# PhilippBongartz/RepeatResolver

Hardware: AMD Instinct MI355X
Metric: sum-of-pairs DP cells/sec (higher is better)
Workload: dtype u32

## Files before the change

repeatresolver_amd/csrc/pwr_device.hip:

```cpp
#include <hip/hip_runtime.h>

#include <algorithm>
#include <chrono>
#include <cstdint>
#include <cstdio>
#include <cstdlib>
#include <cstring>
#include <new>
#include <thread>
#include <type_traits>
#include <vector>

#include "pwr.h"

#define PWR_INF 0x40000000u
#define PWR_BIG 0x7fffffff

struct Hdr {
    int W;
    int nslots;
    int nfree;
    int cur;
    int status;
    int stop;
// ... 85 lines not shown
    int fin, active;
    int grow0;
    unsigned long long cells;
};
struct GatherPart;
struct CommitJob {
    int nchg, nev, ndel, first;
    int u0, u1;
    int scanned, pad;
};
struct BatchPlan;
struct CommitEv;
struct JobBufs {
    GatherPart *gpart;
    unsigned gather_tag;
    JobMeta *meta;
    int *way;
    int4 *rec2;
    uint8_t *mark;
    uint8_t *mark2;
    uint32_t *dirs;
    int *newcol;
    int *aux;
    uint4 *desc;
    int wpNW, wpMS;
    unsigned *lastM;
    unsigned long long *gmb;
    SegDesc *seg;
    unsigned *chk;
    int seg_align;
    int src_start;
    int smax, seg_rows, warm_cols;
    int seg_budget, seg_minrows;
    int seg_balance;
    int plan_ahead;
    int hard_rows, hard_up, hard_down;
    int plan_len;
    int plan_gate_rel;
    int spec_inorder;
    int fail_stops;
    int plan_slack, plan_evrate_x100;
    const int *rowids;
    int gstride;
    unsigned tagbase;
    unsigned long long *gtr;
    int trk;
    unsigned trace_tag;
    long long *g64;
    int force64;
    int evcap;
    int gate_v2;
    int *chkdone;
    int check_in_trace, trace_ny;
    int trace_blk;
    int v2_follows, f64_follows;
    int stall_test;
    unsigned long long *diag;
    int njobs_launched;
    int Lmax, colcap, NC;
    size_t dirstride;
    int split_rank, split_world;
    CommitJob *cjob;
    int *chg;
    int *evkey, *evdl;
    int *insidx;
    int *pair_cf, *pair_left;
    BatchPlan *plan;
    CommitEv *sev;
    int *freed;
    unsigned *ticket;
};
#define NOT_MINE(JB, JOB) ((JB).split_world > 1 && (JOB) % (JB).split_world != (JB).split_rank)

#define DPP_ROW_SHR(n) (0x110 + (n))
#define DPP_ROW_BCAST15 0x142
#define DPP_ROW_BCAST31 0x143
#define DPP_WAVE_SHR1 0x138

__device__ __forceinline__ int wave_incl_min(int v)
{
    int t;
    t = __builtin_amdgcn_update_dpp(PWR_BIG, v, DPP_ROW_SHR(1), 0xF, 0xF, false); v = min(v, t);
    t = __builtin_amdgcn_update_dpp(PWR_BIG, v, DPP_ROW_SHR(2), 0xF, 0xF, false); v = min(v, t);
    t = __builtin_amdgcn_update_dpp(PWR_BIG, v, DPP_ROW_SHR(4), 0xF, 0xF, false); v = min(v, t);
    t = __builtin_amdgcn_update_dpp(PWR_BIG, v, DPP_ROW_SHR(8), 0xF, 0xF, false); v = min(v, t);
    t = __builtin_amdgcn_update_dpp(PWR_BIG, v, DPP_ROW_BCAST15, 0xA, 0xF, false); v = min(v, t);
    t = __builtin_amdgcn_update_dpp(PWR_BIG, v, DPP_ROW_BCAST31, 0xC, 0xF, false); v = min(v, t);
    return v;
}
__device__ __forceinline__ int row_incl_min(int v)
{
    int t;
    t = __builtin_amdgcn_update_dpp(PWR_BIG, v, DPP_ROW_SHR(1), 0xF, 0xF, false); v = min(v, t);
    t = __builtin_amdgcn_update_dpp(PWR_BIG, v, DPP_ROW_SHR(2), 0xF, 0xF, false); v = min(v, t);
    t = __builtin_amdgcn_update_dpp(PWR_BIG, v, DPP_ROW_SHR(4), 0xF, 0xF, false); v = min(v, t);
    t = __builtin_amdgcn_update_dpp(PWR_BIG, v, DPP_ROW_SHR(8), 0xF, 0xF, false); v = min(v, t);
    return v;
}
__device__ __forceinline__ unsigned wave_incl_add(unsigned v)
{
    unsigned t;
    t = __builtin_amdgcn_update_dpp(0u, v, DPP_ROW_SHR(1), 0xF, 0xF, false); v += t;
    t = __builtin_amdgcn_update_dpp(0u, v, DPP_ROW_SHR(2), 0xF, 0xF, false); v += t;
    t = __builtin_amdgcn_update_dpp(0u, v, DPP_ROW_SHR(4), 0xF, 0xF, false); v += t;
    t = __builtin_amdgcn_update_dpp(0u, v, DPP_ROW_SHR(8), 0xF, 0xF, false); v += t;
    t = __builtin_amdgcn_update_dpp(0u, v, DPP_ROW_BCAST15, 0xA, 0xF, false); v += t;
// ... 2075 lines not shown
            const int nv = cbit ? (yy << 1) : ((yy << 1) | 1);
            if (phase == 1 && x >= xrec_lo) cnt -= __builtin_amdgcn_readlane(ncreg, x & 63) & 1;
            cnt += nv & 1;
            ncreg = (lane == (x & 63)) ? nv : ncreg;
            yireg = (lane == (x & 63)) ? y : yireg;
            y = cbit ? yy - 1 : yy;
            --x;
            if (x >= 0 && y < 0) { err = 3; break; }
        }
        if (blk * 64 + lane < L && (x < x_top)) { newcol[blk * 64 + lane] = ncreg; yin[blk * 64 + lane] = yireg; }
        if (phase == 0) {
            if (top) {
                if (err) break;
            } else {
                xrec_lo = err ? x + 1 : x_lo;
                if (err == 0) yout_guess = y;
                err = 0;
            }
            if (top) { yout_guess = y; }
        } else {
            if (err) break;
            if (merged && xrec_lo > x_lo) { err = 6; break; }
            if (merged) y = yout_guess;
            yout_guess = y;
        }
    }
    if (lane == 0)
        __hip_atomic_store(&hand[wv], TR_WORD(ttag, err ? 2 : 1, cnt, yout_guess), __ATOMIC_RELAXED, __HIP_MEMORY_SCOPE_AGENT);
    if (err) {
        if (lane == 0) { m->ok = 0; atomicCAS(&st.hdr->status, 0, PWR_ERR_INTERNAL); }
        return;
    }
#ifdef PWR_DIAG
    if (job == 0 && lane == 0 && (wv == 0 || top)) {
        const unsigned long long n_ = __builtin_amdgcn_s_memrealtime();
        unsigned long long *d_ = st.hdr->dbg + (top ? 20 : 16);
        d_[0] += (top ? n_ : tr_t1) - tr_t0; d_[1] += tr_t2 - tr_t1; d_[2] += n_ - (top ? n_ : tr_t2); d_[3] += 1;
    }
#endif
    if (wv == 0 && lane == 0) {
        int tot = cnt;
        for (int c = 1; c < nch; ++c)
            tot += (int)((__hip_atomic_load(&hand[c], __ATOMIC_RELAXED, __HIP_MEMORY_SCOPE_AGENT) >> 24) & 0xffffull);
        m->nnew = tot;
        m->changed = 1;
    }
}

#define TB_W 4
#ifndef TB_C
#define TB_C 32
#endif
#define TB_BROKE 0x1fffffu
#define TB_WORD(TAG, FLAG, CNT, ARR, EXF) (((unsigned long long)((TAG) & 0x3fffu) << 50) | ((unsigned long long)(FLAG) << 48) | ((unsigned long long)((CNT) & 0x7f) << 41) | \
                                           ((unsigned long long)(((ARR) + 1) & 0xfffff) << 21) | (unsigned long long)((EXF) & 0x1fffffu))
#define TB_MAXCOL ((1 << 20) - 4)
__global__ __launch_bounds__(TB_W * 64) void k_trace_blk(DState st, JobBufs jb)
{
    const int job = blockIdx.x, tid = threadIdx.x, lane = tid & 63;
    if (jb.check_in_trace && (int)blockIdx.y >= jb.trace_ny) { seg_check_body(st, jb, job, (int)blockIdx.y - jb.trace_ny + 1, tid); return; }
    JobMeta *m = &jb.meta[job];
    const int L = UNI(m->L);
    if (!m->active || L <= 0 || !m->ok || m->abort || (!jb.check_in_trace && m->segfail) || (m->wide && !jb.f64_follows) || NOT_MINE(jb, job)) return;
    const int nch = (L + TB_C - 1) / TB_C;
    const int c = nch - 1 - UNI((int)blockIdx.y * TB_W + (tid >> 6));
    if (c < 0) return;
    unsigned long long *const hand = jb.gtr + (size_t)job * jb.trk;
    const unsigned ttag = jb.trace_tag & 0x3fffu;
    const int W = UNI(m->W), B = st.B, H = st.H, RS = jb.NC, lo = UNI(m->lo);
    const int *way = jb.way + (size_t)job * jb.Lmax;
    const uint32_t *dirs = jb.dirs + (size_t)job * jb.dirstride;
    const unsigned *lastM = jb.lastM + (size_t)job * jb.NC;
    int *newcol = jb.newcol + (size_t)job * jb.Lmax;
    int *yin = jb.aux + (size_t)job * jb.Lmax;
    const int x_lo = c * TB_C, x_top = min(L, x_lo + TB_C) - 1;
    const bool top = c == nch - 1;
    const int wcur = way[min(x_lo + lane, L - 1)];
    int ncreg = 0, yireg = 0;
    int xrec_lo = x_top + 1;
    int cnt = 0, err = 0, yexit = 0;
    bool broke = false;

    auto pass = [&](int y0, const bool check_merge, bool &merged) __attribute__((always_inline)) {
        int x = x_top, y = y0;
        int gcur = -1, yb = 0;
        uint32_t win[4] = {0, 0, 0, 0};
        int gpre = -1, ybpre = 0;
        uint32_t pre[4] = {0, 0, 0, 0};
        merged = false;
        int e = 0;
        while (x >= x_lo && !e) {
            x = UNI(x); y = UNI(y); gcur = UNI(gcur); yb = UNI(yb); gpre = UNI(gpre); ybpre = UNI(ybpre); cnt = UNI(cnt);
            while ((x >> 4) == gcur && x >= x_lo) {
                if (check_merge && x >= xrec_lo && __builtin_amdgcn_readlane(yireg, x & (TB_C - 1)) == y) { merged = true; break; }
                const int af = max(0, __builtin_amdgcn_readlane(wcur, x & (TB_C - 1)) - H);
                const int ycf = min(y, af + min(B, W - af) - 1);
                if (y < af || ycf < yb || ycf > yb + 255) break;
                const int q0 = (ycf - yb) >> 6, shf = 15 - (x & 15);
                const uint32_t wq = q0 == 0 ? win[0] : q0 == 1 ? win[1] : q0 == 2 ? win[2] : win[3];
                const int cy = yb + 64 * q0 + lane;
                const unsigned long long mk = __ballot(cy <= ycf && cy >= af && !((wq >> shf) & 1u));
                if (!mk) break;
                const int t = 63 - __builtin_clzll(mk);
                const int yy = yb + 64 * q0 + t;
                const int cb = (int)((__ballot((wq >> (16 + shf)) & 1u) >> t) & 1ull);
                const int nv = (yy << 1) | (cb ^ 1);
                if (x >= xrec_lo) cnt -= __builtin_amdgcn_readlane(ncreg, x & (TB_C - 1)) & 1;
                cnt += nv & 1;
                ncreg = (lane == (x & (TB_C - 1))) ? nv : ncreg;
                yireg = (lane == (x & (TB_C - 1))) ? y : yireg;
                y = yy - cb;
                --x;
                if (x >= 0 && y < 0) { e = 3; break; }
            }
            if (merged || e || x < x_lo) break;
            if (check_merge && x >= xrec_lo && __builtin_amdgcn_readlane(yireg, x & (TB_C - 1)) == y) { merged = true; break; }
            const int a = max(0, __builtin_amdgcn_readlane(wcur, x & (TB_C - 1)) - H);
            const int Bx = min(B, W - a);
            if (y < a) { e = 1; break; }
            int yc = min(y, a + Bx - 1);
            const int g = x >> 4, sh = 15 - (x & 15);
            int found = -1, cbit = 0;
            for (;;) {
                if (g != gcur || yc < yb || yc > yb + 255) {
                    if (gpre == g && yc >= ybpre + 96 && yc <= ybpre + 255) {
#pragma unroll
                        for (int q = 0; q < 4; ++q) win[q] = pre[q];
                        yb = ybpre;
                    } else {
                        const int want = max(lo, yc - 191);
#pragma unroll
                        for (int q = 0; q < 4; ++q) win[q] = dirs[(size_t)g * RS + (want + 64 * q + lane - lo) % RS];
                        yb = want;
                    }
                    gcur = g;
                    if (g > (x_lo >> 4)) {
                        gpre = g - 1; ybpre = max(lo, yb - 56);
#pragma unroll
                        for (int q = 0; q < 4; ++q) pre[q] = dirs[(size_t)(g - 1) * RS + (ybpre + 64 * q + lane - lo) % RS];
                    }
                }
                {
                    const int q0 = (yc - yb) >> 6;
                    const uint32_t wq = q0 == 0 ? win[0] : q0 == 1 ? win[1] : q0 == 2 ? win[2] : win[3];
                    const int cy = yb + 64 * q0 + lane;
                    const unsigned long long mk = __ballot(cy <= yc && cy >= a && !((wq >> sh) & 1u));
                    if (mk) {
                        const int t = 63 - __builtin_clzll(mk);
                        found = yb + 64 * q0 + t;
                        const unsigned long long ck = __ballot((wq >> (16 + sh)) & 1u);
                        cbit = (int)((ck >> t) & 1ull);
                    } else {
#pragma unroll
                        for (int q = 2; q >= 0; --q) {
                            if (found < 0 && q < q0) {
                                const int cy2 = yb + 64 * q + lane;
                                const unsigned long long mk2 = __ballot(cy2 >= a && !((win[q] >> sh) & 1u));
                                if (mk2) {
                                    const int t = 63 - __builtin_clzll(mk2);
                                    found = yb + 64 * q + t;
                                    const unsigned long long ck = __ballot((win[q] >> (16 + sh)) & 1u);
                                    cbit = (int)((ck >> t) & 1ull);
                                }
                            }
                        }
                    }
                }
                if (found >= 0) break;
                if (yb <= a) { e = 2; break; }
                yc = yb - 1;
            }
            if (e) break;
            const int yy = found;
            const int nv = cbit ? (yy << 1) : ((yy << 1) | 1);
            if (x >= xrec_lo) cnt -= __builtin_amdgcn_readlane(ncreg, x & (TB_C - 1)) & 1;
            cnt += nv & 1;
            ncreg = (lane == (x & (TB_C - 1))) ? nv : ncreg;
            yireg = (lane == (x & (TB_C - 1))) ? y : yireg;
            y = cbit ? yy - 1 : yy;
            --x;
            if (x >= 0 && y < 0) { e = 3; break; }
        }
        if (!merged) xrec_lo = e ? min(xrec_lo, x + 1) : x_lo;
        if (!e && !merged) yexit = y;
        return e;
    };
#define TB_POST(FLAG, ARR) if (lane == 0) __hip_atomic_store(&hand[c], TB_WORD(ttag, FLAG, cnt, ARR, broke ? TB_BROKE : (unsigned)(yexit + 1)), __ATOMIC_RELAXED, __HIP_MEMORY_SCOPE_AGENT);

    bool merged = false;
#ifdef PWR_DIAG
    const unsigned long long tb_t0 = __builtin_amdgcn_s_memrealtime();
    unsigned long long tb_t1 = tb_t0;
    int tb_looks = 0, tb_retr = 0;
#endif
    if (top) {
        const int wx = UNI(way[L - 1]);
        const int a = max(0, wx - H), Bx = min(B, W - a);
        int ylow = max(-1, wx - H) + 1;
        if (ylow > W - 1) ylow = W - 1;
        unsigned long long key = ~0ull;
        {
            constexpr int EN = (PWR_MAX_BANDWIDTH + 63) / 64;
            const int y0_ = max(ylow, a) + lane;
            unsigned ev[EN];
#pragma unroll
            for (int i = 0; i < EN; ++i) { const int yy = y0_ + 64 * i; ev[i] = yy < a + Bx ? lastM[(yy - lo) % RS] : 0xffffffffu; }
#pragma unroll
            for (int i = 0; i < EN; ++i) {
                const int yy = y0_ + 64 * i;
                const unsigned long long k2 = yy < a + Bx ? (((unsigned long long)ev[i] << 32) | (unsigned)(~(unsigned)yy)) : ~0ull;
                key = k2 < key ? k2 : key;
            }
        }
        for (int o = 32; o > 0; o >>= 1) {
            const unsigned long long other = __shfl_xor(key, o);
            key = other < key ? other : key;
        }
        const unsigned vmin = (unsigned)(key >> 32);
        int entry = (key == ~0ull) ? -1 : (int)(~(unsigned)key);
        if (a + B <= W - 1) {
            const unsigned lastval = lastM[(a + B - 1 - lo) % RS];
            if (entry < 0 || lastval <= vmin) entry = W - 1;
        }
        entry = UNI(entry);
        if (lane == 0) m->entry = entry;
        err = entry < 0 ? 4 : pass(entry, false, merged);
    } else {
        int arr = UNI(way[x_top + 1]) - 1;
        broke = pass(arr, false, merged) != 0;
        TB_POST(1, arr)
#ifdef PWR_DIAG
        tb_t1 = __builtin_amdgcn_s_memrealtime();
#endif
        for (int look = 0; look < (1 << 16) && !err; ++look) {
#ifdef PWR_DIAG
            tb_looks += 1;
#endif
            int t = c + 1;
            int verdict = 0;
            int bad = -1;
// ... 14 lines not shown
                unsigned ex_up = (unsigned)__shfl_down((int)ex_j, 1);
                if (lane == 63) {
                    const int j2 = min(t + 64, nch - 1);
                    int s2 = 0;
                    for (int spin = 0; spin < TR_SPIN_LIMIT; ++spin) {
                        wn = __hip_atomic_load(&hand[j2], __ATOMIC_RELAXED, __HIP_MEMORY_SCOPE_AGENT);
                        s2 = ((unsigned)(wn >> 50) == ttag) ? (int)((wn >> 48) & 3ull) : 0;
                        if (s2) break;
                        __builtin_amdgcn_s_sleep(1);
                    }
                    ex_up = s2 == 0 || s2 == 3 ? 0u : ((unsigned)wn & 0x1fffffu);
                }
                const bool valid = t + lane <= nch - 1;
                const bool fin = valid && st_j == 2;
                const bool cons = valid && (st_j == 2 || (t + lane < nch - 1 && ar_j == ex_up));
                if (t == c + 1) ex_first = (unsigned)__builtin_amdgcn_readlane((int)ex_j, 0);
                const unsigned long long mfin = __ballot(fin), mbad = __ballot(valid && !cons);
                const int ffin = mfin ? __builtin_ctzll(mfin) : 64, fbad = mbad ? __builtin_ctzll(mbad) : 64;
                if (ffin < 64 && ffin <= fbad) verdict = 1;
                else if (fbad < 64) {
                    verdict = 2; bad = t + fbad;
                    wbad = ((unsigned long long)(unsigned)__builtin_amdgcn_readlane((int)(w >> 32), fbad) << 32) | (unsigned)__builtin_amdgcn_readlane((int)w, fbad);
                }
                else t += 64;
            }
            if (err) break;
            if (ex_first == TB_BROKE) {
                if (verdict == 1) { err = 6; break; }
            } else if ((int)ex_first - 1 != arr) {
                arr = (int)ex_first - 1;
#ifdef PWR_DIAG
                tb_retr += 1;
#endif
                const int e1 = pass(arr, true, merged);
                if (e1) broke = true;
                else if (merged) { if (xrec_lo > x_lo) broke = true; }
                else broke = false;
                TB_POST(1, arr)
                continue;
            } else if (verdict == 1) break;
            for (int spin = 0; spin < TR_SPIN_LIMIT; ++spin) {
                const unsigned long long w = __hip_atomic_load(&hand[bad], __ATOMIC_RELAXED, __HIP_MEMORY_SCOPE_AGENT);
                if (UNI((unsigned)w) != (unsigned)wbad || UNI((unsigned)(w >> 32)) != (unsigned)(wbad >> 32)) break;
                if (spin == TR_SPIN_LIMIT - 1) { err = 5; break; }
                __builtin_amdgcn_s_sleep(1);
            }
        }
        if (!err && broke) err = 6;
        if (!err) { TB_POST(2, arr) }
    }
    if (lane < TB_C && x_lo + lane < L) { newcol[x_lo + lane] = ncreg; yin[x_lo + lane] = yireg; }
    if (__ballot(lane < TB_C && x_lo + lane < L && ncreg != (wcur << 1)) != 0ull && lane == 0) __hip_atomic_store(&m->changed, 1, __ATOMIC_RELAXED, __HIP_MEMORY_SCOPE_AGENT);
    if (top || err) {
        if (lane == 0)
            __hip_atomic_store(&hand[c], TB_WORD(ttag, err ? 3 : 2, cnt, 0, (unsigned)(yexit + 1)), __ATOMIC_RELAXED, __HIP_MEMORY_SCOPE_AGENT);
    }
#ifdef PWR_DIAG
    if (job == 0 && lane == 0) {
        const unsigned long long n_ = __builtin_amdgcn_s_memrealtime();
        if (tb_retr) atomicAdd(&st.hdr->dbg[24], (unsigned long long)tb_retr);
        if (c == 0 || top) {
            unsigned long long *d_ = st.hdr->dbg + (top ? 20 : 16);
            d_[0] += (top ? n_ : tb_t1) - tb_t0; d_[1] += n_ - (top ? n_ : tb_t1); d_[3] += 1;
            if (c == 0) { st.hdr->dbg[25] += (unsigned long long)tb_looks; st.hdr->dbg[26] += (unsigned long long)nch; }
        }
    }
#endif
    if (err) {
        if (lane == 0) {
            bool failed = false;
            if (jb.check_in_trace && seg_check_applies(st, jb, job, m)) {
                const int want = m->nseg - 1;
                for (unsigned spin = 0; spin < (1u << 22) && __hip_atomic_load(&jb.chkdone[job], __ATOMIC_ACQUIRE, __HIP_MEMORY_SCOPE_AGENT) < want; ++spin) __builtin_amdgcn_s_sleep(8);
                failed = __hip_atomic_load(&m->segfail, __ATOMIC_RELAXED, __HIP_MEMORY_SCOPE_AGENT) != 0;
            }
            if (!failed) { m->ok = 0; atomicCAS(&st.hdr->status, 0, PWR_ERR_INTERNAL); }
        }
        return;
    }
    if (c == 0) {
        int tot = 0;
        for (int j = lane; j < nch; j += 64)
            tot += (int)((__hip_atomic_load(&hand[j], __ATOMIC_RELAXED, __HIP_MEMORY_SCOPE_AGENT) >> 41) & 0x7full);
        for (int o = 32; o > 0; o >>= 1) tot += __shfl_xor(tot, o);
        if (lane == 0) m->nnew = tot;
    }
#undef TB_POST
}

#define COMMIT_NT 1024
#define EVCAP 1024
#define MAXJ 128
#define CS_G 16
#define CA_G 32

__device__ __forceinline__ int row_symbol(const uint8_t *mk, int y, int lo, int y0, int y1)
{
    if (y < y0 || y > y1) return 5;
    const int v = mk[y - lo];
    return v == 7 ? 5 : (v ? v - 1 : 4);
}

enum { V_NONE = 0, V_COMMIT, V_STALE, V_STOP_NOTOK, V_STOP_GROW, V_STOP_WIDE, V_STOP_ABORT, V_STOP_SEGFAIL, V_EMPTY, V_AFTER_STOP };
struct BatchPlan {
    int idle;
    int ncommit, nnew, ndel, nev;
// ... 787 lines not shown

#define HIPC(call)                                                                     \
    do {                                                                               \
        hipError_t e_ = (call);                                                        \
        if (e_ != hipSuccess) {                                                        \
            fprintf(stderr, "pwr: %s failed: %s\n", #call, hipGetErrorString(e_));    \
            return PWR_ERR_DEVICE;                                                     \
        }                                                                              \
    } while (0)

struct pwr_ctx {
    int T = 0, B = 0, H = 0, device = 0;
    int W_host = 0;
    std::vector<unsigned char> text;
    bool on_device = false;
    DState st{};
    JobBufs jb{};
    int njobs = 0;
    int *d_jobrows = nullptr;
    int *d_rowids = nullptr;
    std::vector<int> ids, pos_lo;
    unsigned long long *d_score = nullptr;
    hipStream_t stream = nullptr;
    std::vector<int> rowlen;
    long long sumL = 0;
    int Lmax = 0;
    int window = 3;
    double batch_ema = 1.0;
    int profile = 0;
    unsigned gather_tag = 0;
    int force64 = 0;
    int evcap = EVCAP;
    int stall_test = 0;
    int par_trace = 2;
    int cap_slack = 8192;
    int spec_len = 6;
    int fill_mode = 4;
    double host_enqueue_s = 0, host_wait_s = 0;
    unsigned host_seq = 0;
    int seen_fallback = 0, seen_need64 = 0;
    unsigned trace_epoch = 0;
    unsigned fill_epoch = 0;
    int wave_cols = 0;
    int wp_waves = 5;
    int one_wg = 0;
    int one_wg_lds = 0;
    int fill_lds = 0;
    int seg_rows = 160;
    int seg_align = 16;
    int seg_max = 64;
    int seg_budget = 0;
    int seg_minrows = 64;
    int spec_inorder = 64, plan_gate_rel = 1, plan_len = 0;
    int check_in_trace = 1;
    int fail_stops = 1, hard_rows = 1, hard_up_pm = 300, hard_down_pm = 0;
    int plan_slack = PLAN_SLACK, plan_evrate_x100 = (int)(PLAN_EVRATE_MAX * 100.0f);
    int plan_ahead = 1;
    int seg_balance = 0;
    int split_rank = 0, split_world = 1;
    int split_k0 = 0, split_kend = 0;
    int src_start = 1;
    int warm_pct = 190;
    int warm_adapt = 1;
    int warm_min_pct = 100;
    int warm_down_pm = 5, warm_up_pm = 50;
    pwr_stats stats{};
    std::vector<std::pair<hipEvent_t, hipEvent_t>> ev_pool;
    size_t ev_used = 0;
    void *h_hdr = nullptr;
    void *h_ring = nullptr;
    unsigned char *snap_dev = nullptr, *snap_host = nullptr;
    size_t snap_cap = 0;
    hipStream_t snap_stream = nullptr;
    hipEvent_t snap_taken = nullptr, snap_done = nullptr;
    bool snap_busy = false;
    std::vector<void *> allocs;
};
struct pwr_snapshot { pwr_ctx *c; int rows, width; size_t bytes; };

template <class F>
static void par_rows(int T, F f)
{
    unsigned nt = std::min<unsigned>(std::max(1u, std::thread::hardware_concurrency()), 16u);
    nt = (unsigned)std::max(1, std::min<int>((int)nt, T / 64));
    if (nt <= 1) { f(0, T, 0); return; }
    std::vector<std::thread> th;
    for (unsigned t = 0; t < nt; ++t)
        th.emplace_back([=]() { f((int)((long long)T * t / nt), (int)((long long)T * (t + 1) / nt), (int)t); });
    for (auto &x : th) x.join();
}
static unsigned par_threads(int T)
{
    unsigned nt = std::min<unsigned>(std::max(1u, std::thread::hardware_concurrency()), 16u);
    return (unsigned)std::max(1, std::min<int>((int)nt, T / 64));
}

static int code_of_char(unsigned char c)
{
    switch (c) {
    case 'a': case 'A': return 0;
    case 'c': case 'C': return 1;
    case 'g': case 'G': return 2;
    case 't': case 'T': return 3;
    case '-': case '_': return 4;
    case ' ': return 5;
    default: return -1;
// ... 514 lines not shown
    return PWR_OK;
}

static int ensure_device(pwr_ctx *c)
{
    if (c->on_device) { if (hipSetDevice(c->device) != hipSuccess) return PWR_ERR_DEVICE; return PWR_OK; }
    int rc = upload(c);
    if (rc) { free_device(c); return rc; }
    return PWR_OK;
}

static void stats_from_hdr(pwr_ctx *c, const Hdr &h)
{
    c->stats.cells_computed = h.cells_computed;
    c->stats.cells_reference = h.cells_reference;
    c->stats.rows_changed = h.rows_changed;
    c->stats.batches = h.batches;
    c->stats.rows_committed = h.rows_committed;
    c->stats.rows_recomputed = h.rows_recomputed;
    c->stats.rows_wide = h.rows_wide;
    c->stats.stalls = h.stalls;
    c->stats.rows_ahead = h.rows_ahead;
    c->stats.seg_jobs = h.seg_jobs; c->stats.segs = h.segs; c->stats.seg_fails = h.seg_fails;
    c->stats.rows_jumped = h.rows_jumped;
    for (int i = 0; i < 4; ++i) c->stats.reject_reason[i] = h.fail_reason[i];
}

static int check_status(pwr_ctx *c)
{
    Hdr h;
    int rc = read_hdr(c, &h);
    if (rc) return rc;
    stats_from_hdr(c, h);
    return h.status;
}

static int enqueue_front(pwr_ctx *c)
{
    const int n = c->window;
    int rc;
    c->jb.gather_tag = ++c->gather_tag;
    c->jb.rowids = c->d_rowids;
    c->jb.f64_follows = (c->seen_need64 > 0 || c->force64) ? 1 : 0;
    hipLaunchKernelGGL(k_gather_a, dim3(n, GATHER_G), dim3(GATHER_NT), 0, c->stream, c->st, c->jb, c->d_rowids);
    hipLaunchKernelGGL(k_gather_c, dim3(n, GATHER_G + 1), dim3(GATHER_NT), 0, c->stream, c->st, c->jb);
    c->jb.trace_ny = (c->jb.Lmax / TB_C + TB_W) / TB_W;
    c->jb.check_in_trace = (c->check_in_trace && c->fill_mode == 4 && c->par_trace == 2 && c->st.colcap < TB_MAXCOL && c->jb.smax > 1 && c->jb.seg_rows > 0) ? 1 : 0;
    if ((rc = launch_fill(c, n))) return rc;
    if (c->jb.f64_follows) hipLaunchKernelGGL(k_fill64, dim3(n), dim3(F64_NT), 0, c->stream, c->st, c->jb);
    if (c->par_trace) {
        if (++c->trace_epoch >= (1u << 14)) { HIPC(hipMemsetAsync(c->jb.gtr, 0, (size_t)c->njobs * c->jb.trk * 8, c->stream)); c->trace_epoch = 1; }
        c->jb.trace_tag = c->trace_epoch;
        c->jb.trace_blk = (c->par_trace == 2 && c->st.colcap < TB_MAXCOL) ? 1 : 0;
        if (c->jb.trace_blk) hipLaunchKernelGGL(k_trace_blk, dim3(n, c->jb.trace_ny + (c->jb.check_in_trace ? c->jb.smax - 1 : 0)), dim3(TB_W * 64), 0, c->stream, c->st, c->jb);
        else hipLaunchKernelGGL(k_trace_par, dim3(n, TRK / TRW), dim3(TRW * 64), 0, c->stream, c->st, c->jb);
    }
    else { c->jb.trace_blk = 0; hipLaunchKernelGGL(k_trace_wp, dim3(n), dim3(64), 0, c->stream, c->st, c->jb); }
    HIPC(hipGetLastError());
    return PWR_OK;
}

static int enqueue_commit(pwr_ctx *c, Hdr *host_copy, unsigned host_seq)
{
    const int n = c->window;
    hipLaunchKernelGGL(k_commit_scan, dim3(n, CS_G), dim3(COMMIT_NT), 0, c->stream, c->st, c->jb, n);
    hipLaunchKernelGGL(k_commit_apply, dim3(CA_G), dim3(COMMIT_NT), 0, c->stream, c->st, c->jb, n);
    hipLaunchKernelGGL(k_commit_finish, dim3(CA_G), dim3(COMMIT_NT), 0, c->stream, c->st, c->jb, n, c->d_rowids, host_copy, host_seq);
    HIPC(hipGetLastError());
    return PWR_OK;
}

static int enqueue_batch(pwr_ctx *c, Hdr *host_copy, unsigned host_seq)
{
    int rc = enqueue_front(c);
    if (rc) return rc;
    return enqueue_commit(c, host_copy, host_seq);
}

#define PWR_INFLIGHT 3
#define PWR_POLL_LIMIT_S 120

static int slab_init(pwr_ctx *c, int k0, int n)
{
    const int kend = k0 + n;
    int nb = (int)(c->batch_ema + 2.6);
    nb = std::max(1, std::min(nb, std::min(c->window, n)));
    for (int j = 1; j < nb; ++j)
        if (c->rowlen[c->ids[k0 + j]] > c->rowlen[c->ids[k0]] + (int)((long long)c->rowlen[c->ids[k0]] * c->spec_len / 100) + 64) { nb = j; break; }
    const float ema0 = (float)c->batch_ema;
    struct { int next_row, row_end, nb, need_grow, window; } init = {k0, kend, nb, 0, c->window};
    static_assert(sizeof(init) == offsetof(Hdr, fallback) - offsetof(Hdr, next_row), "slab fields of Hdr");
    HIPC(hipMemcpyAsync(&c->st.hdr->ema, &ema0, sizeof(float), hipMemcpyHostToDevice, c->stream));
    HIPC(hipMemcpyAsync(&c->st.hdr->speclen, &c->spec_len, sizeof(int), hipMemcpyHostToDevice, c->stream));
    HIPC(hipMemcpyAsync(&c->st.hdr->next_row, &init, sizeof init, hipMemcpyHostToDevice, c->stream));
    HIPC(hipMemsetAsync(&c->st.hdr->ahead, 0, sizeof(unsigned long long), c->stream));
    HIPC(hipMemsetAsync(c->st.bplan, 0, sizeof(int), c->stream));
    HIPC(hipMemsetAsync(&c->st.hdr->jumpmask, 0, sizeof(unsigned long long), c->stream));
    HIPC(hipStreamSynchronize(c->stream));
    return PWR_OK;
}

static int realign_positions(pwr_ctx *c, int k0, int n, bool resume = false)
{
    if (!c->h_ring) {
        void *p = nullptr;
        if (hipHostMalloc(&p, sizeof(Hdr) * PWR_INFLIGHT, hipHostMallocDefault) != hipSuccess) return PWR_ERR_NOMEM;
// ... 284 lines not shown
extern "C" int pwr_snapshot_wait(pwr_snapshot *sn, const unsigned char **image, size_t *bytes, int *rows, int *width)
{
    if (!sn || !sn->c) return PWR_ERR_ARG;
    if (hipSetDevice(sn->c->device) != hipSuccess) return PWR_ERR_DEVICE;
    if (sn->bytes > 0) HIPC(hipEventSynchronize(sn->c->snap_done));
    if (image) *image = sn->c->snap_host;
    if (bytes) *bytes = sn->bytes;
    if (rows) *rows = sn->rows;
    if (width) *width = sn->width;
    return PWR_OK;
}

extern "C" void pwr_snapshot_free(pwr_snapshot *sn)
{
    if (!sn) return;
    if (sn->c && sn->bytes > 0 && sn->c->snap_done) { (void)hipSetDevice(sn->c->device); (void)hipEventSynchronize(sn->c->snap_done); }
    if (sn->c) sn->c->snap_busy = false;
    delete sn;
}

extern "C" int pwr_trim_ends(pwr_ctx *c)
{
    if (!c) return PWR_ERR_ARG;
    if (!c->on_device) { host_trim(c); return PWR_OK; }
    return PWR_OK;
}

extern "C" int pwr_set_option(pwr_ctx *c, const char *key, long value)
{
    if (!c || !key) return PWR_ERR_ARG;
    if (!strcmp(key, "window")) { if (value < 1 || value > 128 || c->on_device) return PWR_ERR_ARG; c->window = (int)value; return PWR_OK; }
    if (!strcmp(key, "profile")) { if (value < 0 || value > 1000000) return PWR_ERR_ARG; c->profile = (int)value; return PWR_OK; }
    if (!strcmp(key, "spec_len")) { if (value < 0 || value > 100000) return PWR_ERR_ARG; c->spec_len = (int)value; return PWR_OK; }
    if (!strcmp(key, "fill")) { if (c->on_device || (value != 3 && value != 4)) return PWR_ERR_ARG; c->fill_mode = (int)value; return PWR_OK; }
    if (!strcmp(key, "stall_test")) { if (value < 0 || value > 1000000) return PWR_ERR_ARG; c->stall_test = (int)value; return PWR_OK; }
    if (!strcmp(key, "evcap")) { if (value < 0 || value > EVCAP) return PWR_ERR_ARG; c->evcap = (int)value; c->jb.evcap = (int)value; return PWR_OK; }
    if (!strcmp(key, "force64")) { if (value != 0 && value != 1) return PWR_ERR_ARG; c->force64 = (int)value; c->jb.force64 = (int)value; return PWR_OK; }
    if (!strcmp(key, "ptrace")) { if (value < 0 || value > 2) return PWR_ERR_ARG; c->par_trace = (int)value; return PWR_OK; }
    if (!strcmp(key, "slack")) { if (c->on_device || value < 0) return PWR_ERR_ARG; c->cap_slack = (int)value; return PWR_OK; }
    if (!strcmp(key, "fill_epoch")) { if (value < 0 || value >= (1 << 15)) return PWR_ERR_ARG; c->fill_epoch = (unsigned)value; return PWR_OK; }
    if (!strcmp(key, "trace_epoch")) { if (value < 0 || value >= (1 << 14)) return PWR_ERR_ARG; c->trace_epoch = (unsigned)value; return PWR_OK; }
    if (!strcmp(key, "onewg")) { if (value != 0 && value != 1) return PWR_ERR_ARG; c->one_wg = (int)value; return PWR_OK; }
    if (!strcmp(key, "fill_lds")) { if (value < 0 || value > 100000) return PWR_ERR_ARG; c->fill_lds = (int)value; return PWR_OK; }
    if (!strcmp(key, "onewg_lds")) { if (value < 0 || value > 100000) return PWR_ERR_ARG; c->one_wg_lds = (int)value; return PWR_OK; }
    if (!strcmp(key, "seg_rows")) { if (c->on_device || value < 0 || value > 1000000) return PWR_ERR_ARG; c->seg_rows = (int)value; return PWR_OK; }
    if (!strcmp(key, "seg_align")) { if (c->on_device || (value != 16 && value != 32 && value != 64)) return PWR_ERR_ARG; c->seg_align = (int)value; return PWR_OK; }
    if (!strcmp(key, "seg_max")) { if (c->on_device || value < 1 || value > SEG_MAX) return PWR_ERR_ARG; c->seg_max = (int)value; return PWR_OK; }
    if (!strcmp(key, "seg_budget")) { if (value < 0 || value > 100000) return PWR_ERR_ARG; c->seg_budget = (int)value; c->jb.seg_budget = (int)value; return PWR_OK; }
    if (!strcmp(key, "plan_slack")) { if (value < 0 || value > 1000000) return PWR_ERR_ARG; c->plan_slack = (int)value; c->jb.plan_slack = (int)value; return PWR_OK; }
    if (!strcmp(key, "hard_rows")) { if (c->on_device || value < 0 || value > 2) return PWR_ERR_ARG; c->hard_rows = (int)value; return PWR_OK; }
    if (!strcmp(key, "hard_up_pm")) { if (c->on_device || value < 1 || value > 100000) return PWR_ERR_ARG; c->hard_up_pm = (int)value; return PWR_OK; }
    if (!strcmp(key, "hard_down_pm")) { if (c->on_device || value < 0 || value > 100000) return PWR_ERR_ARG; c->hard_down_pm = (int)value; return PWR_OK; }
    if (!strcmp(key, "check_in_trace")) { if (value < 0 || value > 1) return PWR_ERR_ARG; c->check_in_trace = (int)value; return PWR_OK; }
    if (!strcmp(key, "plan_len")) { if (value < 0 || value > 100000) return PWR_ERR_ARG; c->plan_len = (int)value; c->jb.plan_len = (int)value; return PWR_OK; }
    if (!strcmp(key, "plan_gate_rel")) { if (value < 0 || value > 1) return PWR_ERR_ARG; c->plan_gate_rel = (int)value; c->jb.plan_gate_rel = (int)value; return PWR_OK; }
    if (!strcmp(key, "spec_inorder")) { if (value < 0 || value > 64) return PWR_ERR_ARG; c->spec_inorder = (int)value; c->jb.spec_inorder = (int)value; return PWR_OK; }
    if (!strcmp(key, "fail_stops")) { if (value < 0 || value > 1) return PWR_ERR_ARG; c->fail_stops = (int)value; c->jb.fail_stops = (int)value; return PWR_OK; }
    if (!strcmp(key, "plan_evrate_x100")) { if (value < 0 || value > 100000000) return PWR_ERR_ARG; c->plan_evrate_x100 = (int)value; c->jb.plan_evrate_x100 = (int)value; return PWR_OK; }
    if (!strcmp(key, "plan_ahead")) { if (value != 0 && value != 1) return PWR_ERR_ARG; c->plan_ahead = (int)value; c->jb.plan_ahead = (int)value; return PWR_OK; }
    if (!strcmp(key, "seg_balance")) { if (value != 0 && value != 1) return PWR_ERR_ARG; c->seg_balance = (int)value; c->jb.seg_balance = (int)value; return PWR_OK; }
    if (!strcmp(key, "seg_minrows")) { if (value < 16 || value > 100000) return PWR_ERR_ARG; c->seg_minrows = (int)value; c->jb.seg_minrows = (int)value; return PWR_OK; }
    if (!strcmp(key, "src_start")) { if (c->on_device || value < 0 || value > 1) return PWR_ERR_ARG; c->src_start = (int)value; return PWR_OK; }
    if (!strcmp(key, "warm_adapt")) { if (c->on_device || value < 0 || value > 1) return PWR_ERR_ARG; c->warm_adapt = (int)value; return PWR_OK; }
    if (!strcmp(key, "warm_down_pm")) { if (c->on_device || value < 1 || value > 1000) return PWR_ERR_ARG; c->warm_down_pm = (int)value; return PWR_OK; }
    if (!strcmp(key, "warm_up_pm")) { if (c->on_device || value < 1 || value > 10000) return PWR_ERR_ARG; c->warm_up_pm = (int)value; return PWR_OK; }
    if (!strcmp(key, "warm_min_pct")) { if (c->on_device || value < 0 || value > 100000) return PWR_ERR_ARG; c->warm_min_pct = (int)value; return PWR_OK; }
    if (!strcmp(key, "warm_pct")) { if (c->on_device || value < 0 || value > 100000) return PWR_ERR_ARG; c->warm_pct = (int)value; return PWR_OK; }
    if (!strcmp(key, "wave_cols")) { if (c->on_device || (value != 0 && value != 4)) return PWR_ERR_ARG; c->wave_cols = (int)value; return PWR_OK; }
    if (!strcmp(key, "waves")) { if (c->on_device || (value != 3 && value != 4 && value != 5 && value != 8 && value != 9 && value != 17)) return PWR_ERR_ARG; c->wp_waves = (int)value; return PWR_OK; }
    return PWR_ERR_ARG;
}

extern "C" int pwr_get_option(pwr_ctx *c, const char *key, long *value)
{
    if (!c || !key || !value) return PWR_ERR_ARG;
    if (!strcmp(key, "window")) *value = c->window;
    else if (!strcmp(key, "profile")) *value = c->profile;
    else if (!strcmp(key, "spec_len")) *value = c->spec_len;
    else if (!strcmp(key, "fill")) *value = c->fill_mode;
    else if (!strcmp(key, "ptrace")) *value = c->par_trace;
    else if (!strcmp(key, "force64")) *value = c->force64;
    else if (!strcmp(key, "slack")) *value = c->cap_slack;
    else if (!strcmp(key, "waves")) *value = c->wp_waves;
    else if (!strcmp(key, "onewg")) *value = c->one_wg;
    else if (!strcmp(key, "seg_rows")) *value = c->seg_rows;
    else if (!strcmp(key, "seg_max")) *value = c->seg_max;
    else if (!strcmp(key, "seg_budget")) *value = c->seg_budget;
    else if (!strcmp(key, "seg_minrows")) *value = c->seg_minrows;
    else if (!strcmp(key, "seg_balance")) *value = c->seg_balance;
    else if (!strcmp(key, "plan_ahead")) *value = c->plan_ahead;
    else if (!strcmp(key, "plan_slack")) *value = c->plan_slack;
    else if (!strcmp(key, "plan_evrate_x100")) *value = c->plan_evrate_x100;
    else if (!strcmp(key, "fail_stops")) *value = c->fail_stops;
    else if (!strcmp(key, "spec_inorder")) *value = c->spec_inorder;
    else if (!strcmp(key, "plan_gate_rel")) *value = c->plan_gate_rel;
    else if (!strcmp(key, "plan_len")) *value = c->plan_len;
    else if (!strcmp(key, "check_in_trace")) *value = c->check_in_trace;
    else if (!strcmp(key, "hard_rows")) *value = c->hard_rows;
    else if (!strcmp(key, "hard_up_pm")) *value = c->hard_up_pm;
    else if (!strcmp(key, "hard_down_pm")) *value = c->hard_down_pm;
    else if (!strcmp(key, "hard_marked") || !strcmp(key, "hard_fills") || !strcmp(key, "hard_refail")) {
        *value = 0;
        if (c->on_device) { Hdr h; int rc = read_hdr(c, &h); if (rc) return rc; *value = (long)(key[5] == 'm' ? h.hard_marked : key[5] == 'f' ? h.hard_fills : h.hard_refail); }
    }
    else if (!strcmp(key, "evrate_x100")) {
        *value = 0;
        if (c->on_device) { Hdr h; int rc = read_hdr(c, &h); if (rc) return rc; *value = (long)(h.evrate * 100.0f); }
    }
    else if (!strcmp(key, "warm_pct")) *value = c->warm_pct;
    else if (!strcmp(key, "src_start")) *value = c->src_start;
    else if (!strcmp(key, "warm_adapt")) *value = c->warm_adapt;
    else if (!strcmp(key, "host_enqueue_us")) *value = (long)(c->host_enqueue_s * 1e6);
    else if (!strcmp(key, "host_wait_us")) *value = (long)(c->host_wait_s * 1e6);
    else if (!strcmp(key, "warm_now")) {
        if (!c->on_device) *value = c->warm_pct;
        else { Hdr h; int rc = read_hdr(c, &h); if (rc) return rc; *value = h.warm_step > 0 ? (long)(((long long)h.warm_cur * 100 + c->B / 2) / c->B) : c->warm_pct; }
    }
    else if (!strcmp(key, "warm_min_pct")) *value = c->warm_min_pct;
    else if (!strcmp(key, "warm_down_pm")) *value = c->warm_down_pm;
    else if (!strcmp(key, "warm_up_pm")) *value = c->warm_up_pm;
    else return PWR_ERR_ARG;
    return PWR_OK;
}

extern "C" int pwr_get_stats(pwr_ctx *c, pwr_stats *out)
{
    if (!c || !out) return PWR_ERR_ARG;
    if (c->on_device) {
        if (hipSetDevice(c->device) != hipSuccess) return PWR_ERR_DEVICE;
        int rc = check_status(c);
        if (rc) return rc;
        if ((rc = drain_events(c))) return rc;
    }
    *out = c->stats;
    return PWR_OK;
}

extern "C" int pwr_reset_stats(pwr_ctx *c)
{
    if (!c) return PWR_ERR_ARG;
    if (c->on_device) {
        if (hipSetDevice(c->device) != hipSuccess) return PWR_ERR_DEVICE;
        int rc0 = drain_events(c);
        if (rc0) return rc0;
    }
    c->stats = pwr_stats{};
    if (c->on_device) {
        if (hipSetDevice(c->device) != hipSuccess) return PWR_ERR_DEVICE;
        HIPC(hipStreamSynchronize(c->stream));
        HIPC(hipMemset(&c->st.hdr->cells_computed, 0, 16 * sizeof(unsigned long long)));
// ... 79 lines not shown
```

Before: 56.79 billion.

## Precompute per-column prior-path runs in block traceback to skip serial steps

Before the serial traceback starts, each lane checks whether its column's traceback step would simply follow the previous alignment path (the prior 'way' row), using a small lookahead of direction words. These flags are gathered into a ballot mask. During the walk, when the current y matches a lane's predicted value, the whole contiguous run of such columns is taken in one step instead of column by column. The running change counter is replaced with a popcount computed at post time. This adds upfront loads per lane and extra branching, but it can cut the serial per-column cost when the path mostly stays unchanged.

Measured after the change: 57.57 billion, median of 6. 1.01x the previous value.

```diff
diff --git a/repeatresolver_amd/csrc/pwr_device.hip b/repeatresolver_amd/csrc/pwr_device.hip
--- a/repeatresolver_amd/csrc/pwr_device.hip
+++ b/repeatresolver_amd/csrc/pwr_device.hip
@@ -161,6 +161,7 @@
     int gate_v2;
     int *chkdone;
     int check_in_trace, trace_ny;
+    int trace_prior;
     int trace_blk;
     int v2_follows, f64_follows;
     int stall_test;
@@ -2342,6 +2343,7 @@
 #define TB_C 32
 #endif
 #define TB_BROKE 0x1fffffu
+#define TBP_LOOK 8
 #define TB_WORD(TAG, FLAG, CNT, ARR, EXF) (((unsigned long long)((TAG) & 0x3fffu) << 50) | ((unsigned long long)(FLAG) << 48) | ((unsigned long long)((CNT) & 0x7f) << 41) | \
                                            ((unsigned long long)(((ARR) + 1) & 0xfffff) << 21) | (unsigned long long)((EXF) & 0x1fffffu))
 #define TB_MAXCOL ((1 << 20) - 4)
@@ -2371,7 +2373,32 @@
     int cnt = 0, err = 0, yexit = 0;
     bool broke = false;
 
-    auto pass = [&](int y0, const bool check_merge, bool &merged) __attribute__((always_inline)) {
+    const int wnx = __shfl_down(wcur, 1);
+    unsigned long long pmask = 0ull;
+    int ppri = -2;
+    if (jb.trace_prior) {
+        const int xr = x_lo + lane, ya = wnx - 1;
+        const int af = max(0, wcur - H);
+        const int ycf = min(ya, af + min(B, W - af) - 1);
+        bool ok = lane < TB_C && xr < L - 1 && ya >= af && ycf >= wcur && ycf - wcur < TBP_LOOK && wcur >= lo && RS >= TBP_LOOK && (wcur >= 1 || xr == 0);
+        const int i0 = ok ? (wcur - lo) % RS : 0, span = ok ? ycf - wcur : -1;
+        const uint32_t *drow = dirs + (size_t)(min(xr, L - 1) >> 4) * RS;
+        uint32_t pw[TBP_LOOK];
+#pragma unroll
+        for (int k = 0; k < TBP_LOOK; ++k) { const int i = i0 + k; pw[k] = k <= span ? drow[i >= RS ? i - RS : i] : 0u; }
+        const int sh = 15 - (xr & 15);
+        ok = ok && ((pw[0] >> sh) & 0x10001u) == 0x10000u;
+#pragma unroll
+        for (int k = 1; k < TBP_LOOK; ++k) ok = ok && (k > span || ((pw[k] >> sh) & 1u));
+        pmask = __ballot(ok);
+        ppri = ok ? ya : -2;
+    }
+    const bool prior = UNI(jb.trace_prior) != 0;
+    auto ups = [&]() __attribute__((always_inline)) {
+        return (int)__builtin_popcountll(__ballot(lane < TB_C && x_lo + lane >= xrec_lo && x_lo + lane <= x_top && (ncreg & 1)));
+    };
+
+    auto pass_t = [&](auto PRIOR, int y0, const bool check_merge, bool &merged) __attribute__((always_inline)) {
         int x = x_top, y = y0;
         int gcur = -1, yb = 0;
         uint32_t win[4] = {0, 0, 0, 0};
@@ -2379,10 +2406,24 @@
         uint32_t pre[4] = {0, 0, 0, 0};
         merged = false;
         int e = 0;
+        auto take_run = [&]() __attribute__((always_inline)) {
+            if constexpr (!decltype(PRIOR)::value) return false;
+            const int l = x & (TB_C - 1);
+            if (__builtin_amdgcn_readlane(ppri, l) != y) return false;
+            const unsigned long long inv = ~pmask & ((2ull << l) - 1ull);
+            const int l0 = inv ? 64 - __builtin_clzll(inv) : 0;
+            const bool in = lane >= l0 && lane <= l;
+            ncreg = in ? (wcur << 1) : ncreg;
+            yireg = in ? wnx - 1 : yireg;
+            y = __builtin_amdgcn_readlane(wcur, l0) - 1;
+            x = x_lo + l0 - 1;
+            return true;
+        };
         while (x >= x_lo && !e) {
-            x = UNI(x); y = UNI(y); gcur = UNI(gcur); yb = UNI(yb); gpre = UNI(gpre); ybpre = UNI(ybpre); cnt = UNI(cnt);
+            x = UNI(x); y = UNI(y); gcur = UNI(gcur); yb = UNI(yb); gpre = UNI(gpre); ybpre = UNI(ybpre);
             while ((x >> 4) == gcur && x >= x_lo) {
                 if (check_merge && x >= xrec_lo && __builtin_amdgcn_readlane(yireg, x & (TB_C - 1)) == y) { merged = true; break; }
+                if (take_run()) continue;
                 const int af = max(0, __builtin_amdgcn_readlane(wcur, x & (TB_C - 1)) - H);
                 const int ycf = min(y, af + min(B, W - af) - 1);
                 if (y < af || ycf < yb || ycf > yb + 255) break;
@@ -2395,8 +2436,6 @@
                 const int yy = yb + 64 * q0 + t;
                 const int cb = (int)((__ballot((wq >> (16 + shf)) & 1u) >> t) & 1ull);
                 const int nv = (yy << 1) | (cb ^ 1);
-                if (x >= xrec_lo) cnt -= __builtin_amdgcn_readlane(ncreg, x & (TB_C - 1)) & 1;
-                cnt += nv & 1;
                 ncreg = (lane == (x & (TB_C - 1))) ? nv : ncreg;
                 yireg = (lane == (x & (TB_C - 1))) ? y : yireg;
                 y = yy - cb;
@@ -2405,6 +2444,7 @@
             }
             if (merged || e || x < x_lo) break;
             if (check_merge && x >= xrec_lo && __builtin_amdgcn_readlane(yireg, x & (TB_C - 1)) == y) { merged = true; break; }
+            if (take_run()) continue;
             const int a = max(0, __builtin_amdgcn_readlane(wcur, x & (TB_C - 1)) - H);
             const int Bx = min(B, W - a);
             if (y < a) { e = 1; break; }
@@ -2463,8 +2503,6 @@
             if (e) break;
             const int yy = found;
             const int nv = cbit ? (yy << 1) : ((yy << 1) | 1);
-            if (x >= xrec_lo) cnt -= __builtin_amdgcn_readlane(ncreg, x & (TB_C - 1)) & 1;
-            cnt += nv & 1;
             ncreg = (lane == (x & (TB_C - 1))) ? nv : ncreg;
             yireg = (lane == (x & (TB_C - 1))) ? y : yireg;
             y = cbit ? yy - 1 : yy;
@@ -2475,7 +2513,10 @@
         if (!e && !merged) yexit = y;
         return e;
     };
-#define TB_POST(FLAG, ARR) if (lane == 0) __hip_atomic_store(&hand[c], TB_WORD(ttag, FLAG, cnt, ARR, broke ? TB_BROKE : (unsigned)(yexit + 1)), __ATOMIC_RELAXED, __HIP_MEMORY_SCOPE_AGENT);
+    auto pass = [&](int y0, const bool check_merge, bool &merged) __attribute__((always_inline)) {
+        return prior ? pass_t(std::true_type{}, y0, check_merge, merged) : pass_t(std::false_type{}, y0, check_merge, merged);
+    };
+#define TB_POST(FLAG, ARR) cnt = ups(); if (lane == 0) __hip_atomic_store(&hand[c], TB_WORD(ttag, FLAG, cnt, ARR, broke ? TB_BROKE : (unsigned)(yexit + 1)), __ATOMIC_RELAXED, __HIP_MEMORY_SCOPE_AGENT);
 
     bool merged = false;
 #ifdef PWR_DIAG
@@ -2596,6 +2637,7 @@
     if (lane < TB_C && x_lo + lane < L) { newcol[x_lo + lane] = ncreg; yin[x_lo + lane] = yireg; }
     if (__ballot(lane < TB_C && x_lo + lane < L && ncreg != (wcur << 1)) != 0ull && lane == 0) __hip_atomic_store(&m->changed, 1, __ATOMIC_RELAXED, __HIP_MEMORY_SCOPE_AGENT);
     if (top || err) {
+        cnt = ups();
         if (lane == 0)
             __hip_atomic_store(&hand[c], TB_WORD(ttag, err ? 3 : 2, cnt, 0, (unsigned)(yexit + 1)), __ATOMIC_RELAXED, __HIP_MEMORY_SCOPE_AGENT);
     }
@@ -3489,6 +3531,7 @@
     int seg_budget = 0;
     int seg_minrows = 64;
     int spec_inorder = 64, plan_gate_rel = 1, plan_len = 0;
+    int trace_prior = 1;
     int check_in_trace = 1;
     int fail_stops = 1, hard_rows = 1, hard_up_pm = 300, hard_down_pm = 0;
     int plan_slack = PLAN_SLACK, plan_evrate_x100 = (int)(PLAN_EVRATE_MAX * 100.0f);
@@ -4109,6 +4152,7 @@
         if (++c->trace_epoch >= (1u << 14)) { HIPC(hipMemsetAsync(c->jb.gtr, 0, (size_t)c->njobs * c->jb.trk * 8, c->stream)); c->trace_epoch = 1; }
         c->jb.trace_tag = c->trace_epoch;
         c->jb.trace_blk = (c->par_trace == 2 && c->st.colcap < TB_MAXCOL) ? 1 : 0;
+        c->jb.trace_prior = c->trace_prior;
         if (c->jb.trace_blk) hipLaunchKernelGGL(k_trace_blk, dim3(n, c->jb.trace_ny + (c->jb.check_in_trace ? c->jb.smax - 1 : 0)), dim3(TB_W * 64), 0, c->stream, c->st, c->jb);
         else hipLaunchKernelGGL(k_trace_par, dim3(n, TRK / TRW), dim3(TRW * 64), 0, c->stream, c->st, c->jb);
     }
@@ -4499,6 +4543,7 @@
     if (!strcmp(key, "hard_up_pm")) { if (c->on_device || value < 1 || value > 100000) return PWR_ERR_ARG; c->hard_up_pm = (int)value; return PWR_OK; }
     if (!strcmp(key, "hard_down_pm")) { if (c->on_device || value < 0 || value > 100000) return PWR_ERR_ARG; c->hard_down_pm = (int)value; return PWR_OK; }
     if (!strcmp(key, "check_in_trace")) { if (value < 0 || value > 1) return PWR_ERR_ARG; c->check_in_trace = (int)value; return PWR_OK; }
+    if (!strcmp(key, "trace_prior")) { if (value < 0 || value > 1) return PWR_ERR_ARG; c->trace_prior = (int)value; return PWR_OK; }
     if (!strcmp(key, "plan_len")) { if (value < 0 || value > 100000) return PWR_ERR_ARG; c->plan_len = (int)value; c->jb.plan_len = (int)value; return PWR_OK; }
     if (!strcmp(key, "plan_gate_rel")) { if (value < 0 || value > 1) return PWR_ERR_ARG; c->plan_gate_rel = (int)value; c->jb.plan_gate_rel = (int)value; return PWR_OK; }
     if (!strcmp(key, "spec_inorder")) { if (value < 0 || value > 64) return PWR_ERR_ARG; c->spec_inorder = (int)value; c->jb.spec_inorder = (int)value; return PWR_OK; }
@@ -4543,6 +4588,7 @@
     else if (!strcmp(key, "plan_gate_rel")) *value = c->plan_gate_rel;
     else if (!strcmp(key, "plan_len")) *value = c->plan_len;
     else if (!strcmp(key, "check_in_trace")) *value = c->check_in_trace;
+    else if (!strcmp(key, "trace_prior")) *value = c->trace_prior;
     else if (!strcmp(key, "hard_rows")) *value = c->hard_rows;
     else if (!strcmp(key, "hard_up_pm")) *value = c->hard_up_pm;
     else if (!strcmp(key, "hard_down_pm")) *value = c->hard_down_pm;
```
